# maturk/dn-splatter

Hardware: AMD Instinct MI355X
Metric: fwd+bwd frames/sec @1M Gaussians 1080p; HBM GB/s vs roofline (higher is better)
Workload: dtype f32; 1 GPU; c2: 1000000 random-init Gaussians, 1 camera/GPU 1920x1080, SH degree 3 + expected depth + per-Gaussian normals (7 channels, fused one-pass, post-ops in HIP), fx=fy=1200.0, orbit r=8, closed-form 3-NN scale init, random dense cotangents; scene=reference_init, N=1000000, pixels=2073600, bin_policy=deferred, parallelism=single GPU

## Files before the change

### dn-splatter_amd/csrc/binning.hip

```cpp

#include "splat_common.h"
#include "bin_ranges.h"

namespace {

constexpr int RS_THREADS = 256;
#ifndef DNS_RS_ITEMS_I
#define DNS_RS_ITEMS_I 16
#endif
constexpr int RS_ITEMS_I = DNS_RS_ITEMS_I;
#ifndef DNS_RS_ITEMS_N
#define DNS_RS_ITEMS_N 8
#endif
constexpr int RS_ITEMS_N = DNS_RS_ITEMS_N;
constexpr int RS_ITEMS_N_LARGE = 2 * DNS_RS_ITEMS_N;
constexpr int RS_LARGE_N = 1 << 22;
inline int rs_items_n(int N) { return N >= RS_LARGE_N ? RS_ITEMS_N_LARGE : RS_ITEMS_N; }
#ifndef DNS_TI_THREADS
#define DNS_TI_THREADS 512
#endif
constexpr int TI_THREADS = DNS_TI_THREADS;
constexpr int TI_ITEMS = RS_THREADS * RS_ITEMS_I / TI_THREADS;
static_assert(TI_THREADS * TI_ITEMS == RS_THREADS * RS_ITEMS_I && TI_THREADS % DNS_WAVE == 0 && TI_THREADS >= 256, "tile-pass chunk");
constexpr int RS_DIGITS = 256;

constexpr int SC_THREADS = 256;
constexpr int SC_ITEMS = 8;
constexpr int SC_CHUNK = SC_THREADS * SC_ITEMS;

__device__ __forceinline__ uint32_t lane_id() { return threadIdx.x & (DNS_WAVE - 1); }

__device__ __forceinline__ uint32_t wave_incl_scan(uint32_t v)
{
#pragma unroll
    for (int off = 1; off < DNS_WAVE; off <<= 1) {
        uint32_t t = __shfl_up(v, off, DNS_WAVE);
        if ((int)lane_id() >= off) v += t;
    }
    return v;
}

template <int NW = 4>
__device__ __forceinline__ uint32_t block_incl_scan(uint32_t v, uint32_t *lds_wave , uint32_t &total)
{
    const int w = threadIdx.x / DNS_WAVE;
    uint32_t inc = wave_incl_scan(v);
    if (lane_id() == DNS_WAVE - 1) lds_wave[w] = inc;
    __syncthreads();
    uint32_t base = 0, tot = 0;
#pragma unroll
    for (int i = 0; i < NW; ++i) {
        uint32_t s = lds_wave[i];
        if (i < w) base += s;
        tot += s;
    }
    total = tot;
    __syncthreads();
    return inc + base;
}
__device__ __forceinline__ uint32_t block_incl_scan_256(uint32_t v, uint32_t *lds_wave , uint32_t &total)
{
    return block_incl_scan<4>(v, lds_wave, total);
}

__device__ __forceinline__ uint32_t depth_key(const int32_t *__restrict__ radii, const float *__restrict__ depths, uint32_t g)
{
    return radii[g] > 0 ? __float_as_uint(depths[g]) : 0xFFFFFFFFu;
}

struct __align__(16) EmitRec {
    uint32_t gid;
    uint32_t start;
    uint32_t base_tile;
    uint32_t bw;
};
struct GenArgs {
    const EmitRec *__restrict__ jrec;
    const uint32_t *__restrict__ cum;
    const uint32_t *__restrict__ chunk_first;
    int N, tw;
    int exact;
    const uint32_t *__restrict__ n_ranked;
};

constexpr int gen_pad(int i) { return i + (i >> 5); }
// ... 325 lines not shown
        }
        const uint32_t prior = wave_cnt[w][d];
        const uint32_t below = __popcll(m & lt_mask);
        rnk[r] = prior + below;
        if (valid && below == 0) wave_cnt[w][d] = prior + __popcll(m);
    }
    __syncthreads();
    uint32_t n_out = n_valid;
    {
        const bool has_digit = threadIdx.x < ND;
        uint32_t cw[NW];
        uint32_t cnt = 0;
#pragma unroll
        for (int i = 0; i < NW; ++i) {
            cw[i] = has_digit ? wave_cnt[i][threadIdx.x] : 0u;
            cnt += cw[i];
        }
        uint32_t t2;
        const uint32_t linc = block_incl_scan<NW>(cnt, lds_wave, t2);
        const uint32_t ls = linc - cnt;
        if (FIRST) n_out = t2;
        if (has_digit) {
            dstart[threadIdx.x] = ls;
            uint32_t run = ls;
#pragma unroll
            for (int i = 0; i < NW; ++i) {
                wave_loc[i][threadIdx.x] = run;
                run += cw[i];
            }
        }
        const uint32_t tot = pre_tot;
        const uint32_t ginc = block_incl_scan<NW>(tot, lds_wave, t2);
        if (has_digit) gbase[threadIdx.x] = is_digit ? (ginc - tot) + pre_tab : 0u;
        if (FIRST && count_out && blockIdx.x == 0 && threadIdx.x == 0) *count_out = t2;
    }
    __syncthreads();
#pragma unroll
    for (int r = 0; r < ITEMS; ++r) {
        const uint32_t idx = wave_start + r * DNS_WAVE + lane;
        if (FIRST ? ((live >> r) & 1u) != 0u : idx < n) {
            const uint32_t d = (key[r] >> shift) & DMASK;
            const uint32_t lpos = wave_loc[w][d] + rnk[r];
            keys_s[lpos] = (K)key[r];
            vals_s[lpos] = val[r];
        }
    }
    __syncthreads();
    if constexpr (BOXG) {
        uint32_t dsts[ITEMS], vs[ITEMS];
        int2 bx[ITEMS];
#pragma unroll
        for (int r = 0; r < ITEMS; ++r) {
            const uint32_t i = min((uint32_t)(r * TH + threadIdx.x), n_out - 1u);
            const uint32_t d = ((uint32_t)keys_s[i] >> shift) & DMASK;
            dsts[r] = gbase[d] + (i - dstart[d]);
            vs[r] = vals_s[i];
        }
#pragma unroll
        for (int r = 0; r < ITEMS; ++r) bx[r] = box_in[vs[r]];
#pragma unroll
        for (int r = 0; r < ITEMS; ++r)
            if ((uint32_t)(r * TH + threadIdx.x) < n_out) {
                vals_out[dsts[r]] = vs[r];
                box_out[dsts[r]] = bx[r];
                tiles_out[dsts[r]] = ((uint32_t)bx[r].y & 0xffffu) * ((uint32_t)bx[r].y >> 16);
            }
        return;
    }
#pragma unroll
    for (int r = 0; r < ITEMS; ++r) {
        const uint32_t i = r * TH + threadIdx.x;
        if (i < n_out) {
            const uint32_t k = keys_s[i];
            const uint32_t d = (k >> shift) & DMASK;
            const uint32_t dst = gbase[d] + (i - dstart[d]);
            if (!LAST) keys_out[dst] = (K)k;
            vals_out[dst] = vals_s[i];
            if (LAST && (i == 0 || (uint32_t)keys_s[i - 1] != k)) atomicMin(&tile_first[k], (int32_t)dst);
            if (LAST && tile_end && (i + 1 == n_valid || (uint32_t)keys_s[i + 1] != k)) atomicMax(&tile_end[k], (int32_t)dst + 1);
        }
    }
}

template <bool BOXES>
__global__ __launch_bounds__(SC_THREADS) void scan_sums_kernel(int N, const uint32_t *__restrict__ n_ptr,
                                                               const uint32_t *__restrict__ order,
                                                               const int32_t *__restrict__ tiles,
                                                               uint32_t *__restrict__ sums, uint32_t *__restrict__ tiles_sorted,
                                                               const int2 *__restrict__ boxes = nullptr,
                                                               int2 *__restrict__ boxes_sorted = nullptr)
{
    __shared__ uint32_t lds_wave[4];
    const int n = (int)min(*n_ptr, (uint32_t)N);
    const int base = blockIdx.x * SC_CHUNK + threadIdx.x * SC_ITEMS;
    uint32_t s = 0;
    if (blockIdx.x * SC_CHUNK < n) {
        uint32_t o[SC_ITEMS], t[SC_ITEMS];
        [[maybe_unused]] int2 bx[SC_ITEMS];
#pragma unroll
        for (int i = 0; i < SC_ITEMS; ++i) o[i] = order[min(base + i, n - 1)];
#pragma unroll
        for (int i = 0; i < SC_ITEMS; ++i) {
            if (BOXES) {
                bx[i] = boxes[o[i]];
                t[i] = ((uint32_t)bx[i].y & 0xffffu) * ((uint32_t)bx[i].y >> 16);
            } else t[i] = (uint32_t)tiles[o[i]];
        }
#pragma unroll
        for (int i = 0; i < SC_ITEMS; ++i)
            if (base + i < n) {
                s += t[i];
                tiles_sorted[base + i] = t[i];
                if (BOXES) boxes_sorted[base + i] = bx[i];
            }
    }
    uint32_t tot;
    block_incl_scan_256(s, lds_wave, tot);
    if (threadIdx.x == 0) sums[blockIdx.x] = tot;
}

__global__ __launch_bounds__(SC_THREADS) void scan_sums_sorted_kernel(int N, const uint32_t *__restrict__ n_ptr,
                                                                      const uint32_t *__restrict__ tiles_sorted, uint32_t *__restrict__ sums)
{
    __shared__ uint32_t lds_wave[4];
    const int n = (int)min(*n_ptr, (uint32_t)N);
    const int base = blockIdx.x * SC_CHUNK + threadIdx.x * SC_ITEMS;
    uint32_t s = 0;
#pragma unroll
    for (int i = 0; i < SC_ITEMS; ++i)
        if (base + i < n) s += tiles_sorted[base + i];
    uint32_t tot;
    block_incl_scan_256(s, lds_wave, tot);
    if (threadIdx.x == 0) sums[blockIdx.x] = tot;
}

struct EmitPrep {
    EmitRec *__restrict__ jrec;
    uint32_t *__restrict__ chunk_first;
    int nb_chunks, chunk;
    int n_per_cam, tile_size, tw, th;
    const float *__restrict__ means2d;
    const int32_t *__restrict__ radii;
    const float4 *__restrict__ splats;
    const int2 *__restrict__ boxes;
    const int2 *__restrict__ boxes_sorted;
};

__device__ __forceinline__ void emit_record(const EmitPrep &ep, int N, uint32_t j, uint32_t gid, uint32_t start, uint32_t end)
{
    EmitRec r;
    r.gid = gid; r.start = start;
    const uint32_t cam_tiles = (ep.n_per_cam < N) ? (gid / (uint32_t)ep.n_per_cam) * (uint32_t)(ep.tw * ep.th) : 0u;
    if (ep.boxes) {
        const int2 b = ep.boxes_sorted ? ep.boxes_sorted[j] : ep.boxes[gid];
        r.bw = (uint32_t)b.y & 0xffffu;
        r.base_tile = (uint32_t)b.x + cam_tiles;
    } else {
        int x0, y0, x1, y1;
        if (ep.splats) {
            const float4 r0 = ep.splats[(size_t)gid * 4], r1 = ep.splats[(size_t)gid * 4 + 1];
            dns_snug_tile_bbox(r0.x, r0.y, r0.z, r0.w, r1.x, r1.y, (float)ep.radii[gid], ep.tile_size, ep.tw, ep.th, x0, y0, x1, y1);
        } else
            dns_tile_bbox(ep.means2d[2 * gid], ep.means2d[2 * gid + 1], (float)ep.radii[gid], ep.tile_size, ep.tw, ep.th, x0, y0, x1, y1);
        r.base_tile = (uint32_t)(y0 * ep.tw + x0) + cam_tiles;
        r.bw = (uint32_t)(x1 - x0);
    }
// ... 29 lines not shown
    for (int c = threadIdx.x; c < (int)blockIdx.x; c += SC_THREADS) before += sums[c];
    uint32_t tot_before;
    block_incl_scan_256(before, lds_wave, tot_before);
    uint32_t tot;
    uint32_t inc = block_incl_scan_256(s, lds_wave, tot);
    uint32_t run = tot_before + inc - s;
#pragma unroll
    for (int i = 0; i < SC_ITEMS; ++i) {
        int j = base + i;
        run += v[i];
        if (j < n) {
            cum[j] = run;
            if (j == n - 1) {
                *total_u32 = run; *total_i64 = (int64_t)run;
                if (total_max) atomicMax(reinterpret_cast<unsigned long long *>(total_max), (unsigned long long)run);
            }
        }
    }
}

__global__ __launch_bounds__(256) void emit_prep_kernel(int N, const uint32_t *__restrict__ n_ptr, const uint32_t *__restrict__ order,
                                                        const uint32_t *__restrict__ cum, EmitPrep ep)
{
    const uint32_t j = blockIdx.x * blockDim.x + threadIdx.x;
    if (j >= min(*n_ptr, (uint32_t)N)) return;
    const uint32_t end = cum[j], start = j ? cum[j - 1] : 0u;
    if (end > start) emit_record(ep, N, j, order[j], start, end);
}

constexpr int TO_THREADS = 1024;
__global__ __launch_bounds__(TO_THREADS) void tile_offsets_fill_kernel(int n_tiles, int32_t *__restrict__ offsets)
{
    __shared__ int32_t seg_min[TO_THREADS];
    const int total = n_tiles + 1;
    const int per = (total + TO_THREADS - 1) / TO_THREADS;
    const int lo = threadIdx.x * per, hi = min(lo + per, total);
    int32_t m = 0x7fffffff;
    for (int i = hi - 1; i >= lo; --i) m = min(m, offsets[i]);
    seg_min[threadIdx.x] = m;
    __syncthreads();
    for (int off = 1; off < TO_THREADS; off <<= 1) {
        const int32_t other = threadIdx.x + off < TO_THREADS ? seg_min[threadIdx.x + off] : 0x7fffffff;
        __syncthreads();
        seg_min[threadIdx.x] = min(seg_min[threadIdx.x], other);
        __syncthreads();
    }
    int32_t run = threadIdx.x + 1 < TO_THREADS ? seg_min[threadIdx.x + 1] : 0x7fffffff;
    for (int i = hi - 1; i >= lo; --i) {
        run = min(run, offsets[i]);
        offsets[i] = run;
    }
}

__global__ __launch_bounds__(256) void isect_ids_kernel(int n_tiles, int tile_bits, const int32_t *__restrict__ offsets,
                                                        const int32_t *__restrict__ flatten_ids,
                                                        const float *__restrict__ depths, int64_t *__restrict__ isect_ids,
                                                        int64_t cap)
{
    const int t = blockIdx.x;
    const int64_t cam = t / n_tiles, local = t % n_tiles;
    const int64_t hi = (cam << (32 + tile_bits)) | (local << 32);
    const int s = offsets[t], e = offsets[t + 1];
    for (int i = s + threadIdx.x; i < e && i < cap; i += blockDim.x) {
        const uint32_t bits = __float_as_uint(depths[flatten_ids[i]]);
        isect_ids[i] = hi | (int64_t)bits;
    }
}

constexpr int MAX_CHUNKS = (int)((0x80000000ull + RS_THREADS * RS_ITEMS_I - 1) / (RS_THREADS * RS_ITEMS_I));

struct BinWs {
    uint32_t *key_a, *key_b, *val_a, *val_b;
    uint32_t *cum;
    uint32_t *tiles_sorted;
    int2 *boxes_sorted;
    EmitRec *jrec;
    uint32_t *chunk_first;
    uint32_t *tab_n;
    uint32_t *totals;
    uint32_t *sums;
    uint32_t *total;
    uint32_t *status;
    uint32_t *n_ranked;
    uint32_t *tkey_b, *tval_b;
    uint32_t *tkey_c, *tval_c;
    uint32_t *tab_i;
    int nb_n, nb_i, nb_scan;
    size_t bytes;
};

inline size_t align_up(size_t v, size_t a) { return (v + a - 1) / a * a; }

BinWs carve(void *ws, int N, int64_t cap)
{
    BinWs b{};
    b.nb_n = (N + RS_THREADS * rs_items_n(N) - 1) / (RS_THREADS * rs_items_n(N));
    b.nb_i = (int)((cap + RS_THREADS * RS_ITEMS_I - 1) / (RS_THREADS * RS_ITEMS_I));
    b.nb_scan = (N + SC_CHUNK - 1) / SC_CHUNK;
    if (b.nb_n < 1) b.nb_n = 1;
    if (b.nb_i < 1) b.nb_i = 1;
    if (b.nb_scan < 1) b.nb_scan = 1;
    size_t off = 0;
    char *base = (char *)ws;
    auto take = [&](size_t elems) {
        uint32_t *p = (uint32_t *)(base + off);
        off += align_up(elems * sizeof(uint32_t), 256);
        return p;
    };
    size_t n = (size_t)(N > 0 ? N : 1), c = (size_t)(cap > 0 ? cap : 1);
    b.key_a = take(n); b.key_b = take(n); b.val_a = take(n); b.val_b = take(n);
    b.cum = take(n);
    b.tiles_sorted = take(n);
    b.boxes_sorted = reinterpret_cast<int2 *>(take(2 * n));
    b.jrec = reinterpret_cast<EmitRec *>(take(4 * n));
    b.chunk_first = take(MAX_CHUNKS);
    b.tab_n = take((size_t)RS_DIGITS * b.nb_n);
    b.totals = take((size_t)RS_DIGITS * SC_MAX_SEGS);
    b.sums = take(b.nb_scan);
    b.total = take(1);
    b.status = take(1);
    b.n_ranked = take(1);
    b.tkey_b = take(c); b.tval_b = take(c);
    b.tkey_c = take(c); b.tval_c = take(c);
    b.tab_i = take((size_t)RS_DIGITS * b.nb_i);
    b.bytes = off;
    return b;
}

int tile_bits(int n_tiles);

template <typename K, int ITEMS, int TH = RS_THREADS>
void radix_pass(hipStream_t stream, const K *ka, const uint32_t *va, K *kb, uint32_t *vb, const uint32_t *n_ptr,
                uint32_t n_cap, int shift, int dbits, uint32_t *table, uint32_t *totals, int nb, int32_t *tile_first = nullptr,
                const int32_t *radii = nullptr, const float *depths = nullptr, int32_t *init_offsets = nullptr, int n_tiles = 0,
                int32_t *tile_end = nullptr, const GenArgs *gen = nullptr, uint32_t *status = nullptr, uint32_t *count_out = nullptr,
                const int2 *box_in = nullptr, int2 *box_out = nullptr, uint32_t *tiles_out = nullptr)
{
    const uint32_t mask = (1u << dbits) - 1u;
    int segs, seg_len;
    scan_segments(nb, segs, seg_len);
    if (radii) {
        hipLaunchKernelGGL((radix_hist_kernel<K, ITEMS, true, false, TH>), dim3(nb), dim3(TH), 0, stream, ka, n_ptr, n_cap, shift, mask, table, nb, radii, depths);
        hipLaunchKernelGGL(radix_scan_kernel, dim3((1 << dbits) * segs), dim3(SC_THREADS), 0, stream, table, nb, totals, segs, seg_len);
        hipLaunchKernelGGL((radix_scatter_kernel<K, false, 8, ITEMS, true, false, TH>), dim3(nb), dim3(TH), 0, stream, ka, va, kb, vb,
                           n_ptr, n_cap, shift, table, totals, nb, tile_first, radii, depths, (int32_t *)nullptr, GenArgs{}, count_out,
                           (const int2 *)nullptr, (int2 *)nullptr, (uint32_t *)nullptr, segs, seg_len);
        return;
    }
    const GenArgs g = gen ? *gen : GenArgs{};
    if (gen && DNS_GEN_HIST_RANGES && shift == 0 && TH > RS_DIGITS)
        hipLaunchKernelGGL((radix_hist_ranges_kernel<ITEMS, (TH > RS_DIGITS ? TH : 2 * RS_DIGITS)>), dim3(nb), dim3(TH), 0, stream, n_ptr, n_cap, dbits,
                           table, nb, init_offsets, n_tiles, init_offsets ? tile_end : nullptr, g, status);
    else if (gen)
        hipLaunchKernelGGL((radix_hist_kernel<K, ITEMS, false, true, TH>), dim3(nb), dim3(TH), 0, stream, ka, n_ptr, n_cap, shift, mask,
                           table, nb, (const int32_t *)nullptr, (const float *)nullptr, init_offsets, n_tiles, init_offsets ? tile_end : nullptr, g, status);
    else
        hipLaunchKernelGGL((radix_hist_kernel<K, ITEMS, false, false, TH>), dim3(nb), dim3(TH), 0, stream, ka, n_ptr, n_cap, shift, mask, table, nb,
                           (const int32_t *)nullptr, (const float *)nullptr, init_offsets, n_tiles, init_offsets ? tile_end : nullptr, g, status);
    hipLaunchKernelGGL(radix_scan_kernel, dim3((1 << dbits) * segs), dim3(SC_THREADS), 0, stream, table, nb, totals, segs, seg_len);
    if constexpr (sizeof(K) == 4) {
        if (box_in && !gen && !tile_first && dbits == 8) {
            hipLaunchKernelGGL((radix_scatter_kernel<K, false, 8, ITEMS, false, false, TH, true>), dim3(nb), dim3(TH), 0, stream, ka, va, kb, vb,
                               n_ptr, n_cap, shift, table, totals, nb, tile_first, (const int32_t *)nullptr, (const float *)nullptr,
                               (int32_t *)nullptr, GenArgs{}, (uint32_t *)nullptr, box_in, box_out, tiles_out, segs, seg_len);
            return;
        }
    }
#define DNS_SCATTER3(B, L, G)                                                                                               \
    hipLaunchKernelGGL((radix_scatter_kernel<K, L, B, ITEMS, false, G, TH>), dim3(nb), dim3(TH), 0, stream, ka, va, kb, vb,    \
                       n_ptr, n_cap, shift, table, totals, nb, tile_first, (const int32_t *)nullptr, (const float *)nullptr, \
                       tile_end, g, (uint32_t *)nullptr, (const int2 *)nullptr, (int2 *)nullptr, (uint32_t *)nullptr, segs, seg_len)
#define DNS_SCATTER(B)                                                                                                      \
    do {                                                                                                                    \
        if (tile_first) { if (gen) DNS_SCATTER3(B, true, true); else DNS_SCATTER3(B, true, false); }                        \
        else { if (gen) DNS_SCATTER3(B, false, true); else DNS_SCATTER3(B, false, false); }                                 \
    } while (0)
    switch (dbits) {
        case 1: DNS_SCATTER(1); break;
        case 2: DNS_SCATTER(2); break;
        case 3: DNS_SCATTER(3); break;
        case 4: DNS_SCATTER(4); break;
        case 5: DNS_SCATTER(5); break;
        case 6: DNS_SCATTER(6); break;
        case 7: DNS_SCATTER(7); break;
        default: DNS_SCATTER(8); break;
    }
#undef DNS_SCATTER
#undef DNS_SCATTER3
}

template <typename K>
void emit_and_sort(hipStream_t stream, const dnsplat_bin_args *a, const BinWs &w, int tw, int th, int n_tiles, uint32_t cap)
{
    K *kb = reinterpret_cast<K *>(w.tkey_b), *kc = reinterpret_cast<K *>(w.tkey_c);
    uint32_t *vb = w.tval_b, *vc = w.tval_c;
    const int n_cam = a->n_cameras > 1 ? a->n_cameras : 1;
    const int bits = tile_bits(n_tiles);
    const int passes = (bits + 7) / 8;
    GenArgs g;
    g.jrec = w.jrec; g.cum = w.cum; g.chunk_first = w.chunk_first;
    g.N = a->N; g.tw = tw; g.n_ranked = w.n_ranked;
    g.exact = (tw <= 256 && (int64_t)n_cam * tw * th <= 65536) ? 1 : 0;
    const K *ka = nullptr;
    const uint32_t *va = nullptr;
// ... 47 lines not shown
    d.totals = take((size_t)RS_DIGITS * SC_MAX_SEGS);
    d.count = take(1);
    d.bytes = off;
    return d;
}

__global__ __launch_bounds__(256) void det_iota_kernel(const int64_t *__restrict__ n_isects, uint32_t cap, uint32_t *__restrict__ vals,
                                                       uint32_t *__restrict__ count)
{
    const uint32_t n = (uint32_t)min((int64_t)cap, max((int64_t)0, *n_isects));
    if (blockIdx.x == 0 && threadIdx.x == 0) *count = n;
    for (uint32_t i = blockIdx.x * blockDim.x + threadIdx.x; i < n; i += gridDim.x * blockDim.x) vals[i] = i;
}

__global__ __launch_bounds__(256) void det_reduce_kernel(const uint32_t *__restrict__ count, const uint32_t *__restrict__ keys,
                                                         const uint32_t *__restrict__ vals, const float *__restrict__ partials,
                                                         size_t cap, int n_records, float *__restrict__ v_splats)
{
    const uint32_t n = *count;
    const uint32_t i = (uint32_t)(((size_t)blockIdx.x * blockDim.x + threadIdx.x) >> 4);
    const int col = threadIdx.x & 15;
    if (i >= n) return;
    const uint32_t g = keys[i];
    if ((i > 0 && keys[i - 1] == g) || g >= (uint32_t)n_records) return;
    double acc = 0.0;
    for (uint32_t j = i; j < n && keys[j] == g; ++j) {
        const size_t e = vals[j];
        acc += (double)partials[e * DNS_REC + col];
        acc += (double)partials[(cap + e) * DNS_REC + col];
    }
    v_splats[(size_t)g * DNS_REC + col] = (float)acc;
}

}

extern "C" size_t dnsplat_det_workspace_bytes(int64_t capacity)
{
    if (capacity < 0) return 0;
    return det_carve(nullptr, capacity).bytes;
}

extern "C" int dnsplat_det_reduce(const dnsplat_det_args *a, dnsplat_stream_t stream_)
{
    if (!a || a->n_records < 0 || a->capacity < 0 || a->capacity > 0x7fffffffLL) return DNSPLAT_ERR_INVALID_ARG;
    if (a->capacity == 0 || a->n_records == 0) return DNSPLAT_OK;
    if (!a->n_isects || !a->flatten_ids || !a->partials || !a->v_splats || !a->workspace) return DNSPLAT_ERR_INVALID_ARG;
    if (a->workspace_bytes < det_carve(nullptr, a->capacity).bytes) return DNSPLAT_ERR_WORKSPACE;
    hipStream_t stream = (hipStream_t)stream_;
    const DetWs w = det_carve(a->workspace, a->capacity);
    const uint32_t cap = (uint32_t)a->capacity;
    hipLaunchKernelGGL(det_iota_kernel, dim3(1024), dim3(256), 0, stream, a->n_isects, cap, w.val_a, w.count);
    int bits = 1;
    while ((1ll << bits) < (long long)a->n_records) ++bits;
    const int passes = (bits + 7) / 8;
    const uint32_t *ka = reinterpret_cast<const uint32_t *>(a->flatten_ids);
    uint32_t *va = w.val_a, *kb = w.key_a, *vb = w.val_b;
    for (int pass = 0; pass < passes; ++pass) {
        radix_pass<uint32_t, RS_ITEMS_N>(stream, ka, va, kb, vb, w.count, cap, 8 * pass, 8, w.table, w.totals, w.nb);
        ka = kb; va = vb;
        kb = (kb == w.key_a) ? w.key_b : w.key_a;
        vb = (vb == w.val_b) ? w.val_a : w.val_b;
    }
    const size_t groups = (size_t)cap;
    hipLaunchKernelGGL(det_reduce_kernel, dim3((unsigned)((groups * 16 + 255) / 256)), dim3(256), 0, stream, w.count, ka, va, a->partials,
                       (size_t)a->capacity, a->n_records, a->v_splats);
    DNS_CHECK_LAUNCH();
    return DNSPLAT_OK;
}

extern "C" size_t dnsplat_bin_workspace_bytes(int32_t N, int64_t isect_capacity, int32_t n_tiles)
{
    (void)n_tiles;
    if (N < 0 || isect_capacity < 0) return 0;
    return carve(nullptr, N, isect_capacity).bytes;
}

extern "C" size_t dnsplat_bin_status_offset(int32_t N, int64_t isect_capacity)
{
    if (N < 0 || isect_capacity < 0) return 0;
    const BinWs w = carve(nullptr, N, isect_capacity);
    return (size_t)((char *)w.status - (char *)nullptr);
}

static int check_bin(const dnsplat_bin_args *a)
{
    if (!a) return DNSPLAT_ERR_INVALID_ARG;
    if (a->N < 0 || a->width <= 0 || a->height <= 0 || a->tile_size <= 0) return DNSPLAT_ERR_INVALID_ARG;
    if (a->n_cameras < 0 || (a->n_cameras > 1 && a->N % a->n_cameras != 0)) return DNSPLAT_ERR_INVALID_ARG;
    if (a->isect_capacity < 0 || a->isect_capacity > 0x7fffffffLL) return DNSPLAT_ERR_INVALID_ARG;
    if (!a->n_isects || !a->workspace) return DNSPLAT_ERR_INVALID_ARG;
    if (a->N > 0 && (!a->means2d || !a->radii || !a->depths || !a->tiles_per_gauss)) return DNSPLAT_ERR_INVALID_ARG;
    if (a->workspace_bytes < carve(nullptr, a->N, a->isect_capacity).bytes) return DNSPLAT_ERR_WORKSPACE;
    return DNSPLAT_OK;
}

extern "C" int dnsplat_bin_prepare(const dnsplat_bin_args *a, dnsplat_stream_t stream_)
{
    int rc = check_bin(a);
    if (rc != DNSPLAT_OK) return rc;
    hipStream_t stream = (hipStream_t)stream_;
    BinWs w = carve(a->workspace, a->N, a->isect_capacity);
    const int N = a->N;
    if (a->tight_tiles && !a->splats && !a->tile_boxes && N > 0) return DNSPLAT_ERR_INVALID_ARG;
    if (N == 0) {
        if (hipMemsetAsync(a->n_isects, 0, sizeof(int64_t), stream) != hipSuccess) return DNSPLAT_ERR_LAUNCH;
        if (hipMemsetAsync(w.total, 0, sizeof(uint32_t), stream) != hipSuccess) return DNSPLAT_ERR_LAUNCH;
    } else {
        const uint32_t n_u32 = (uint32_t)N;
        uint32_t *ka = w.key_a, *kb = w.key_b, *va = w.val_a, *vb = w.val_b;
        const int2 *boxes = reinterpret_cast<const int2 *>(a->tile_boxes);
        static const bool box_gather = [] { const char *e = getenv("DNSPLAT_BIN_BOX_GATHER"); return !(e && e[0] == '0'); }();
        const bool sorted_boxes = boxes && box_gather;
        static const bool box_fold = [] { const char *e = getenv("DNSPLAT_BIN_BOX_FOLD"); return !(e && e[0] == '0'); }();
        const bool fold = sorted_boxes && box_fold;
        for (int pass = 0; pass < 4; ++pass) {
            const int shift = 8 * pass;
            const bool fold_here = fold && pass == 3;
            if (rs_items_n(N) == RS_ITEMS_N_LARGE)
                radix_pass<uint32_t, RS_ITEMS_N_LARGE>(stream, ka, va, kb, vb, pass == 0 ? nullptr : w.n_ranked, n_u32, shift, 8, w.tab_n, w.totals,
                                                       w.nb_n, nullptr, pass == 0 ? a->radii : nullptr, pass == 0 ? a->depths : nullptr, nullptr, 0,
                                                       nullptr, nullptr, nullptr, pass == 0 ? w.n_ranked : nullptr,
                                                       fold_here ? boxes : nullptr, w.boxes_sorted, w.tiles_sorted);
            else
                radix_pass<uint32_t, RS_ITEMS_N>(stream, ka, va, kb, vb, pass == 0 ? nullptr : w.n_ranked, n_u32, shift, 8, w.tab_n, w.totals,
                                                 w.nb_n, nullptr, pass == 0 ? a->radii : nullptr, pass == 0 ? a->depths : nullptr, nullptr, 0,
                                                 nullptr, nullptr, nullptr, pass == 0 ? w.n_ranked : nullptr,
                                                 fold_here ? boxes : nullptr, w.boxes_sorted, w.tiles_sorted);
            uint32_t *t = ka; ka = kb; kb = t;
            t = va; va = vb; vb = t;
        }
        if (fold)
            hipLaunchKernelGGL(scan_sums_sorted_kernel, dim3(w.nb_scan), dim3(SC_THREADS), 0, stream, N, w.n_ranked, w.tiles_sorted, w.sums);
        else if (sorted_boxes)
            hipLaunchKernelGGL(scan_sums_kernel<true>, dim3(w.nb_scan), dim3(SC_THREADS), 0, stream, N, w.n_ranked, w.val_a, a->tiles_per_gauss,
                               w.sums, w.tiles_sorted, boxes, w.boxes_sorted);
        else
            hipLaunchKernelGGL(scan_sums_kernel<false>, dim3(w.nb_scan), dim3(SC_THREADS), 0, stream, N, w.n_ranked, w.val_a, a->tiles_per_gauss,
                               w.sums, w.tiles_sorted);
        EmitPrep ep;
        ep.jrec = w.jrec; ep.chunk_first = w.chunk_first; ep.nb_chunks = MAX_CHUNKS; ep.chunk = RS_THREADS * RS_ITEMS_I;
        ep.n_per_cam = N / (a->n_cameras > 1 ? a->n_cameras : 1);
        ep.tile_size = a->tile_size;
        ep.tw = dns_tiles_w(a->width, a->tile_size); ep.th = dns_tiles_h(a->height, a->tile_size);
        ep.means2d = a->means2d; ep.radii = a->radii;
        ep.splats = a->tight_tiles ? reinterpret_cast<const float4 *>(a->splats) : nullptr;
        ep.boxes = boxes;
        ep.boxes_sorted = sorted_boxes ? w.boxes_sorted : nullptr;
        hipLaunchKernelGGL(scan_final_kernel, dim3(w.nb_scan), dim3(SC_THREADS), 0, stream, N, w.n_ranked, w.val_a,
                           (const int32_t *)w.tiles_sorted, w.sums, w.cum, w.total, a->n_isects, a->n_isects_max);
        hipLaunchKernelGGL(emit_prep_kernel, dim3((N + 255) / 256), dim3(256), 0, stream, N, w.n_ranked, w.val_a, w.cum, ep);
        DNS_CHECK_LAUNCH();
    }
    if (a->n_isects_host) {
        if (hipMemcpyAsync(a->n_isects_host, a->n_isects, sizeof(int64_t), hipMemcpyDeviceToHost, stream) != hipSuccess)
            return DNSPLAT_ERR_LAUNCH;
    }
    return DNSPLAT_OK;
}

extern "C" int dnsplat_bin_emit_sort(const dnsplat_bin_args *a, dnsplat_stream_t stream_)
{
    int rc = check_bin(a);
    if (rc != DNSPLAT_OK) return rc;
    if (!a->tile_offsets || (a->isect_capacity > 0 && !a->flatten_ids)) return DNSPLAT_ERR_INVALID_ARG;
    if (a->tight_tiles && !a->splats && !a->tile_boxes && a->N > 0) return DNSPLAT_ERR_INVALID_ARG;
    hipStream_t stream = (hipStream_t)stream_;
    BinWs w = carve(a->workspace, a->N, a->isect_capacity);
    const int tw = dns_tiles_w(a->width, a->tile_size), th = dns_tiles_h(a->height, a->tile_size);
    const int64_t n_tiles64 = (int64_t)tw * th * (a->n_cameras > 1 ? a->n_cameras : 1);
    if (n_tiles64 > 0x7fffffffLL) return DNSPLAT_ERR_UNSUPPORTED;
    const int n_tiles = (int)n_tiles64;
    const uint32_t cap = (uint32_t)a->isect_capacity;
    if (a->N == 0 || cap == 0) {
        if (hipMemsetAsync(a->tile_offsets, 0, sizeof(int32_t) * (size_t)(n_tiles + 1), stream) != hipSuccess)
            return DNSPLAT_ERR_LAUNCH;
        if (a->tile_ends && hipMemsetAsync(a->tile_ends, 0, sizeof(int32_t) * (size_t)n_tiles, stream) != hipSuccess)
            return DNSPLAT_ERR_LAUNCH;
        return DNSPLAT_OK;
    }
    if (n_tiles <= 0x10000) emit_and_sort<uint16_t>(stream, a, w, tw, th, n_tiles, cap);
    else emit_and_sort<uint32_t>(stream, a, w, tw, th, n_tiles, cap);
    DNS_CHECK_LAUNCH();
    return DNSPLAT_OK;
}

extern "C" int dnsplat_bin_isect_ids(int32_t n_tiles, int32_t n_cameras, const int32_t *tile_offsets,
                                     const int32_t *flatten_ids, const float *depths, int64_t *isect_ids, int64_t capacity,
                                     dnsplat_stream_t stream)
{
    if (n_tiles <= 0 || n_cameras < 0 || !tile_offsets || !isect_ids) return DNSPLAT_ERR_INVALID_ARG;
    if (capacity == 0) return DNSPLAT_OK;
    if (!flatten_ids || !depths) return DNSPLAT_ERR_INVALID_ARG;
    const int n_cam = n_cameras > 1 ? n_cameras : 1;
    int tb = 0;
    while ((n_tiles >> tb) != 0) ++tb;
    hipLaunchKernelGGL(isect_ids_kernel, dim3(n_tiles * n_cam), dim3(256), 0, (hipStream_t)stream, n_tiles, tb, tile_offsets,
                       flatten_ids, depths, isect_ids, capacity);
    DNS_CHECK_LAUNCH();
    return DNSPLAT_OK;
}
```

Before: 476.1 frames/s.

## Sort depths via bucket partition and per-bucket LDS radix sort for mid-size N

For N below the large threshold, replaces the four global 8-bit radix passes over depth keys with a min/max bounds pass, a single histogram+scatter partition into depth buckets, and a per-bucket radix sort in shared memory that also gathers tile boxes. The aim is to cut global memory traffic and kernel launches of the full radix sort. Skewed depth distributions can overflow the LDS cap and fall back to slower in-global LSD passes inside one workgroup.

```diff
diff --git a/dn-splatter_amd/csrc/binning.hip b/dn-splatter_amd/csrc/binning.hip
--- a/dn-splatter_amd/csrc/binning.hip
+++ b/dn-splatter_amd/csrc/binning.hip
@@ -1,6 +1,9 @@
 
+#include <assert.h>
+#include <string.h>
 #include "splat_common.h"
 #include "bin_ranges.h"
+#include "depth_buckets.h"
 
 namespace {
 
@@ -492,6 +495,392 @@
     }
 }
 
+constexpr int DP_THREADS = 256;
+constexpr int DP_ITEMS = 16;
+constexpr int DP_CHUNK = DP_THREADS * DP_ITEMS;
+constexpr int DP_NW = DP_THREADS / DNS_WAVE;
+constexpr int DP_CAP = DNS_DP_CAP;
+constexpr int DP_BOUNDS_WGS = 1024;
+static_assert(DP_BOUNDS_WGS % DP_THREADS == 0, "the partials are reduced in rounds of one per thread");
+#ifndef DNS_DP_BBITS
+#define DNS_DP_BBITS 0
+#endif
+inline int dp_bbits(int N) { return DNS_DP_BBITS ? DNS_DP_BBITS : dns_depth_bucket_bits(N); }
+inline int dp_sub(int N) { const int s = (1 << dp_bbits(N)) >> 10; return s < 1 ? 1 : s; }
+inline int dp_bounds_wgs(int N)
+{
+    const int g = (N + DP_CHUNK - 1) / DP_CHUNK;
+    return g < 1 ? 1 : (g > DP_BOUNDS_WGS ? DP_BOUNDS_WGS : g);
+}
+
+__device__ __forceinline__ void dp_block_minmax(uint32_t &mn, uint32_t &mx, uint32_t *red )
+{
+#pragma unroll
+    for (int off = DNS_WAVE / 2; off > 0; off >>= 1) {
+        mn = min(mn, (uint32_t)__shfl_xor((int)mn, off, DNS_WAVE));
+        mx = max(mx, (uint32_t)__shfl_xor((int)mx, off, DNS_WAVE));
+    }
+    const int w = threadIdx.x / DNS_WAVE;
+    if (lane_id() == 0) { red[2 * w] = mn; red[2 * w + 1] = mx; }
+    __syncthreads();
+#pragma unroll
+    for (int i = 0; i < DP_NW; ++i) { mn = min(mn, red[2 * i]); mx = max(mx, red[2 * i + 1]); }
+    __syncthreads();
+}
+
+__global__ __launch_bounds__(DP_THREADS) void depth_bounds_kernel(const int32_t *__restrict__ radii, const float *__restrict__ depths,
+                                                                  uint32_t n, uint32_t *__restrict__ part)
+{
+    __shared__ uint32_t red[2 * DP_NW];
+    uint32_t mn = 0xFFFFFFFFu, mx = 0u;
+    constexpr int U = 4;
+    for (uint32_t i0 = blockIdx.x * (DP_THREADS * U) + threadIdx.x; i0 < n; i0 += gridDim.x * (DP_THREADS * U)) {
+        int32_t r[U];
+        uint32_t k[U];
+#pragma unroll
+        for (int u = 0; u < U; ++u) {
+            const uint32_t i = min(i0 + u * DP_THREADS, n - 1u);
+            r[u] = radii[i];
+            k[u] = __float_as_uint(depths[i]);
+        }
+#pragma unroll
+        for (int u = 0; u < U; ++u)
+            if (r[u] > 0) { mn = min(mn, k[u]); mx = max(mx, k[u]); }
+    }
+    dp_block_minmax(mn, mx, red);
+    if (threadIdx.x == 0) { part[2 * blockIdx.x] = mn; part[2 * blockIdx.x + 1] = mx; }
+}
+
+template <int BBITS>
+__global__ __launch_bounds__(DP_THREADS) void depth_part_hist_kernel(const int32_t *__restrict__ radii, const float *__restrict__ depths,
+                                                                     uint32_t n, const uint32_t *__restrict__ part, int n_part,
+                                                                     uint32_t *__restrict__ ks, uint32_t *__restrict__ table, int nb,
+                                                                     int sub)
+{
+    constexpr int NB = 1 << BBITS;
+    __shared__ uint32_t hist[NB];
+    __shared__ uint32_t red[2 * DP_NW];
+    uint32_t mn = 0xFFFFFFFFu, mx = 0u;
+    for (int i = threadIdx.x; i < n_part; i += DP_THREADS) { mn = min(mn, part[2 * i]); mx = max(mx, part[2 * i + 1]); }
+    for (int d = threadIdx.x; d < NB; d += DP_THREADS) hist[d] = 0u;
+    dp_block_minmax(mn, mx, red);
+    uint32_t kmin = 0u;
+    int shift = 0;
+    if (mn <= mx) { kmin = mn; shift = dns_depth_bucket_shift(mn, mx, BBITS); }
+    if (blockIdx.x == 0 && threadIdx.x == 0) { ks[0] = kmin; ks[1] = (uint32_t)shift; }
+    for (int c = 0; c < sub; ++c) {
+        const uint32_t base = (blockIdx.x * sub + c) * DP_CHUNK;
+        if (base >= n) break;
+        int32_t r[DP_ITEMS];
+        uint32_t k[DP_ITEMS];
+#pragma unroll
+        for (int i = 0; i < DP_ITEMS; ++i) {
+            const uint32_t idc = min(base + i * DP_THREADS + threadIdx.x, n - 1u);
+            r[i] = radii[idc];
+            k[i] = __float_as_uint(depths[idc]);
+        }
+#pragma unroll
+        for (int i = 0; i < DP_ITEMS; ++i)
+            if (base + i * DP_THREADS + threadIdx.x < n && r[i] > 0) atomicAdd(&hist[dns_depth_bucket(k[i], kmin, shift) & (NB - 1)], 1u);
+    }
+    __syncthreads();
+    for (int d = threadIdx.x; d < NB; d += DP_THREADS) table[(size_t)d * nb + blockIdx.x] = hist[d];
+}
+
+template <int BBITS>
+__global__ __launch_bounds__(DP_THREADS) void depth_part_scatter_kernel(
+    const int32_t *__restrict__ radii, const float *__restrict__ depths, uint32_t n, const uint32_t *__restrict__ ks,
+    uint2 *__restrict__ pairs_out, const uint32_t *__restrict__ table, const uint32_t *__restrict__ totals, int nb, int segs, int seg_len,
+    uint32_t *__restrict__ count_out, uint32_t *__restrict__ bucket_start, int sub)
+{
+    constexpr int NB = 1 << BBITS;
+    constexpr int DPT = NB / DP_THREADS;
+    static_assert(NB % DP_THREADS == 0 && DP_CHUNK <= 0xFFFF, "bucket scan layout / 16-bit chunk-local counts");
+    __shared__ __align__(4) uint16_t wave_cnt[DP_NW][NB];
+    __shared__ uint32_t gbase[NB];
+    __shared__ uint32_t lds_wave[DP_NW];
+    const uint32_t base0 = blockIdx.x * sub * DP_CHUNK;
+    if (base0 >= n) return;
+    const uint32_t kmin = ks[0];
+    const int shift = (int)ks[1];
+    const int w = threadIdx.x / DNS_WAVE;
+    const uint32_t lane = lane_id();
+    const uint64_t lt_mask = (lane == 0) ? 0ull : (~0ull >> (64 - lane));
+    {
+        uint32_t pre_tot[DPT], pre_tab[DPT];
+        const int my_seg = (int)blockIdx.x / seg_len;
+        uint32_t tsum = 0u;
+#pragma unroll
+        for (int q = 0; q < DPT; ++q) {
+            const int d = threadIdx.x * DPT + q;
+            pre_tab[q] = table[(size_t)d * nb + blockIdx.x];
+            pre_tot[q] = 0u;
+            for (int sg = 0; sg < segs; ++sg) {
+                const uint32_t v = totals[d * segs + sg];
+                pre_tot[q] += v;
+                if (sg < my_seg) pre_tab[q] += v;
+            }
+            tsum += pre_tot[q];
+        }
+        uint32_t total;
+        const uint32_t inc = block_incl_scan<DP_NW>(tsum, lds_wave, total);
+        uint32_t run = inc - tsum;
+#pragma unroll
+        for (int q = 0; q < DPT; ++q) {
+            const int d = threadIdx.x * DPT + q;
+            gbase[d] = run + pre_tab[q];
+            if (blockIdx.x == 0) bucket_start[d] = run;
+            run += pre_tot[q];
+        }
+        if (blockIdx.x == 0 && threadIdx.x == 0) { bucket_start[NB] = total; *count_out = total; }
+    }
+    for (int c = 0; c < sub; ++c) {
+        const uint32_t base = base0 + c * DP_CHUNK;
+        if (base >= n) break;
+        {
+            uint32_t *z = reinterpret_cast<uint32_t *>(&wave_cnt[0][0]);
+            for (int i = threadIdx.x; i < DP_NW * NB / 2; i += DP_THREADS) z[i] = 0u;
+        }
+        __syncthreads();
+        const uint32_t wave_start = base + w * (DNS_WAVE * DP_ITEMS);
+        uint32_t key[DP_ITEMS];
+        int32_t rad[DP_ITEMS];
+        uint16_t rnk[DP_ITEMS];
+#pragma unroll
+        for (int r = 0; r < DP_ITEMS; ++r) {
+            const uint32_t idc = min(wave_start + r * DNS_WAVE + lane, n - 1u);
+            rad[r] = radii[idc];
+            key[r] = __float_as_uint(depths[idc]);
+        }
+        uint32_t live = 0u;
+#pragma unroll
+        for (int r = 0; r < DP_ITEMS; ++r) {
+            const uint32_t idx = wave_start + r * DNS_WAVE + lane;
+            const bool valid = idx < n && rad[r] > 0;
+            live |= (valid ? 1u : 0u) << r;
+            const uint32_t d = valid ? (dns_depth_bucket(key[r], kmin, shift) & (NB - 1)) : 0u;
+            uint64_t m = dns_ballot(valid);
+#pragma unroll
+            for (int bit = 0; bit < BBITS; ++bit) {
+                const bool b = (d >> bit) & 1;
+                const uint64_t bal = dns_ballot(b);
+                m &= b ? bal : ~bal;
+            }
+            const uint32_t prior = wave_cnt[w][d];
+            const uint32_t below = __popcll(m & lt_mask);
+            rnk[r] = (uint16_t)(prior + below);
+            if (valid && below == 0) wave_cnt[w][d] = (uint16_t)(prior + __popcll(m));
+        }
+        __syncthreads();
+        uint32_t cnt[DPT];
+#pragma unroll
+        for (int q = 0; q < DPT; ++q) {
+            const int d = threadIdx.x * DPT + q;
+            uint32_t run = 0u;
+#pragma unroll
+            for (int i = 0; i < DP_NW; ++i) {
+                const uint32_t v = wave_cnt[i][d];
+                wave_cnt[i][d] = (uint16_t)run;
+                run += v;
+            }
+            cnt[q] = run;
+        }
+        __syncthreads();
+#pragma unroll
+        for (int r = 0; r < DP_ITEMS; ++r)
+            if ((live >> r) & 1u) {
+                const uint32_t d = dns_depth_bucket(key[r], kmin, shift) & (NB - 1);
+                const uint32_t dst = gbase[d] + wave_cnt[w][d] + rnk[r];
+                pairs_out[dst] = make_uint2(key[r], wave_start + r * DNS_WAVE + lane);
+            }
+        __syncthreads();
+#pragma unroll
+        for (int q = 0; q < DPT; ++q) gbase[threadIdx.x * DPT + q] += cnt[q];
+    }
+}
+
+__device__ __forceinline__ void dp_lsd_pass(const uint2 *src, uint2 *dst, uint32_t n, uint32_t kmin, int sh, int dbits,
+                                            uint32_t *dig_run , uint32_t (*wave_cnt)[256] , uint32_t *lds_wave)
+{
+    static_assert(DP_THREADS == 256, "one thread per digit");
+    const uint32_t mask = (1u << dbits) - 1u;
+    const int w = threadIdx.x / DNS_WAVE;
+    const uint32_t lane = lane_id();
+    const uint64_t lt_mask = (lane == 0) ? 0ull : (~0ull >> (64 - lane));
+    dig_run[threadIdx.x] = 0u;
+#pragma unroll
+    for (int i = 0; i < DP_NW; ++i) wave_cnt[i][threadIdx.x] = 0u;
+    __syncthreads();
+    for (uint32_t i = threadIdx.x; i < n; i += DP_THREADS) atomicAdd(&dig_run[((src[i].x - kmin) >> sh) & mask], 1u);
+    __syncthreads();
+    {
+        const uint32_t v = dig_run[threadIdx.x];
+        uint32_t tot;
+        const uint32_t inc = block_incl_scan<DP_NW>(v, lds_wave, tot);
+        dig_run[threadIdx.x] = inc - v;
+    }
+    __syncthreads();
+    for (uint32_t b0 = 0; b0 < n; b0 += DP_THREADS) {
+        const uint32_t i = b0 + threadIdx.x;
+        const bool valid = i < n;
+        const uint2 p = src[valid ? i : n - 1u];
+        const uint32_t d = valid ? (((p.x - kmin) >> sh) & mask) : 0u;
+        uint64_t m = dns_ballot(valid);
+#pragma unroll
+        for (int bit = 0; bit < 8; ++bit) {
+            const bool b = (d >> bit) & 1;
+            const uint64_t bal = dns_ballot(b);
+            m &= b ? bal : ~bal;
+        }
+        const uint32_t below = __popcll(m & lt_mask);
+        if (valid && below == 0) wave_cnt[w][d] = __popcll(m);
+        __syncthreads();
+        if (valid) {
+            uint32_t pos = dig_run[d] + below;
+#pragma unroll
+            for (int q = 0; q < DP_NW; ++q)
+                if (q < w) pos += wave_cnt[q][d];
+            dst[pos] = p;
+        }
+        __syncthreads();
+        {
+            uint32_t s = 0u;
+#pragma unroll
+            for (int q = 0; q < DP_NW; ++q) { s += wave_cnt[q][threadIdx.x]; wave_cnt[q][threadIdx.x] = 0u; }
+            dig_run[threadIdx.x] += s;
+        }
+        __syncthreads();
+    }
+}
+
+__device__ __forceinline__ void dp_store_bucket(const uint2 *res, uint32_t s, uint32_t n, uint32_t *__restrict__ vals_out,
+                                                const int2 *__restrict__ box_in, int2 *__restrict__ box_out,
+                                                uint32_t *__restrict__ tiles_out)
+{
+    constexpr int U = 4;
+    for (uint32_t i0 = threadIdx.x; i0 < n; i0 += U * DP_THREADS) {
+        uint32_t v[U];
+        int2 bx[U];
+#pragma unroll
+        for (int u = 0; u < U; ++u) v[u] = res[min(i0 + u * DP_THREADS, n - 1u)].y;
+        if (box_in) {
+#pragma unroll
+            for (int u = 0; u < U; ++u) bx[u] = box_in[v[u]];
+        }
+#pragma unroll
+        for (int u = 0; u < U; ++u) {
+            const uint32_t i = i0 + u * DP_THREADS;
+            if (i < n) {
+                vals_out[s + i] = v[u];
+                if (box_in) {
+                    box_out[s + i] = bx[u];
+                    tiles_out[s + i] = ((uint32_t)bx[u].y & 0xffffu) * ((uint32_t)bx[u].y >> 16);
+                }
+            }
+        }
+    }
+}
+
+__device__ __forceinline__ void dp_sort_in_lds(const uint2 *__restrict__ in, uint32_t n, uint32_t kmin, int passes, int dbits, uint2 *buf,
+                                               uint32_t *dig_start , uint32_t (*wave_cnt)[256] , uint32_t *lds_wave)
+{
+    constexpr int ITEMS = DP_CAP / DP_THREADS;
+    const int w = threadIdx.x / DNS_WAVE;
+    const uint32_t lane = lane_id();
+    const uint64_t lt_mask = (lane == 0) ? 0ull : (~0ull >> (64 - lane));
+    const int ipw = (int)((n + DP_THREADS - 1) / DP_THREADS);
+    const uint32_t first = (uint32_t)w * DNS_WAVE * ipw + lane;
+    const uint32_t mask = (1u << dbits) - 1u;
+    uint2 p[ITEMS];
+    uint32_t rnk[ITEMS];
+#pragma unroll
+    for (int r = 0; r < ITEMS; ++r)
+        if (r < ipw) p[r] = in[min(first + r * DNS_WAVE, n - 1u)];
+    if (passes == 0) {
+#pragma unroll
+        for (int r = 0; r < ITEMS; ++r)
+            if (r < ipw && first + r * DNS_WAVE < n) buf[first + r * DNS_WAVE] = p[r];
+    }
+    for (int pass = 0; pass < passes; ++pass) {
+        const int sh = pass * dbits;
+#pragma unroll
+        for (int i = 0; i < DP_NW; ++i) wave_cnt[i][threadIdx.x] = 0u;
+        __syncthreads();
+#pragma unroll
+        for (int r = 0; r < ITEMS; ++r)
+            if (r < ipw) {
+                const bool valid = first + r * DNS_WAVE < n;
+                const uint32_t d = valid ? (((p[r].x - kmin) >> sh) & mask) : 0u;
+                uint64_t m = dns_ballot(valid);
+#pragma unroll
+                for (int bit = 0; bit < 8; ++bit) {
+                    const bool b = (d >> bit) & 1;
+                    const uint64_t bal = dns_ballot(b);
+                    m &= b ? bal : ~bal;
+                }
+                const uint32_t prior = wave_cnt[w][d];
+                const uint32_t below = __popcll(m & lt_mask);
+                rnk[r] = prior + below;
+                if (valid && below == 0) wave_cnt[w][d] = prior + __popcll(m);
+            }
+        __syncthreads();
+        {
+            uint32_t cnt = 0u;
+#pragma unroll
+            for (int i = 0; i < DP_NW; ++i) {
+                const uint32_t c = wave_cnt[i][threadIdx.x];
+                wave_cnt[i][threadIdx.x] = cnt;
+                cnt += c;
+            }
+            uint32_t tot;
+            const uint32_t inc = block_incl_scan<DP_NW>(cnt, lds_wave, tot);
+            dig_start[threadIdx.x] = inc - cnt;
+        }
+        __syncthreads();
+#pragma unroll
+        for (int r = 0; r < ITEMS; ++r)
+            if (r < ipw && first + r * DNS_WAVE < n) {
+                const uint32_t d = ((p[r].x - kmin) >> sh) & mask;
+                buf[dig_start[d] + wave_cnt[w][d] + rnk[r]] = p[r];
+            }
+        __syncthreads();
+        if (pass + 1 < passes) {
+#pragma unroll
+            for (int r = 0; r < ITEMS; ++r)
+                if (r < ipw) p[r] = buf[min(first + r * DNS_WAVE, n - 1u)];
+        }
+    }
+    __syncthreads();
+}
+
+__global__ __launch_bounds__(DP_THREADS) void depth_bucket_sort_kernel(const uint32_t *__restrict__ ks,
+                                                                       const uint32_t *__restrict__ bucket_start, uint2 *pairs_a,
+                                                                       uint2 *pairs_b, uint32_t *__restrict__ vals_out,
+                                                                       const int2 *__restrict__ box_in, int2 *__restrict__ box_out,
+                                                                       uint32_t *__restrict__ tiles_out)
+{
+    __shared__ uint2 buf[DP_CAP];
+    __shared__ uint32_t dig_run[256];
+    __shared__ uint32_t wave_cnt[DP_NW][256];
+    __shared__ uint32_t lds_wave[DP_NW];
+    const uint32_t s = bucket_start[blockIdx.x], n = bucket_start[blockIdx.x + 1] - s;
+    if (n == 0) return;
+    const uint32_t kmin = ks[0];
+    const int shift = (int)ks[1];
+    const int passes = dns_depth_local_passes(shift), dbits = dns_depth_local_bits(shift);
+    if (n <= (uint32_t)DP_CAP) {
+        dp_sort_in_lds(pairs_a + s, n, kmin, passes, dbits, buf, dig_run, wave_cnt, lds_wave);
+        dp_store_bucket(buf, s, n, vals_out, box_in, box_out, tiles_out);
+    } else {
+        uint2 *src = pairs_a + s, *dst = pairs_b + s;
+        for (int p = 0; p < passes; ++p) {
+            dp_lsd_pass(src, dst, n, kmin, p * dbits, dbits, dig_run, wave_cnt, lds_wave);
+            uint2 *t = src; src = dst; dst = t;
+        }
+        dp_store_bucket(src, s, n, vals_out, box_in, box_out, tiles_out);
+    }
+}
+
 template <bool BOXES>
 __global__ __launch_bounds__(SC_THREADS) void scan_sums_kernel(int N, const uint32_t *__restrict__ n_ptr,
                                                                const uint32_t *__restrict__ order,
@@ -687,10 +1076,15 @@
     uint32_t *total;
     uint32_t *status;
     uint32_t *n_ranked;
+    uint32_t *dp_part;
+    uint32_t *dp_ks;
+    uint32_t *dp_start;
+    uint32_t *dp_tab;
+    uint32_t *dp_totals;
     uint32_t *tkey_b, *tval_b;
     uint32_t *tkey_c, *tval_c;
     uint32_t *tab_i;
-    int nb_n, nb_i, nb_scan;
+    int nb_n, nb_i, nb_scan, nb_p;
     size_t bytes;
 };
 
@@ -705,6 +1099,8 @@
     if (b.nb_n < 1) b.nb_n = 1;
     if (b.nb_i < 1) b.nb_i = 1;
     if (b.nb_scan < 1) b.nb_scan = 1;
+    b.nb_p = (N + DP_CHUNK * dp_sub(N) - 1) / (DP_CHUNK * dp_sub(N));
+    if (b.nb_p < 1) b.nb_p = 1;
     size_t off = 0;
     char *base = (char *)ws;
     auto take = [&](size_t elems) {
@@ -725,6 +1121,17 @@
     b.total = take(1);
     b.status = take(1);
     b.n_ranked = take(1);
+    {
+        const size_t B = (size_t)1 << dp_bbits(N), tab = B * b.nb_p;
+        uint32_t *q = b.chunk_first;
+        b.dp_part = q; q += 2 * DP_BOUNDS_WGS;
+        b.dp_ks = q; q += 64;
+        b.dp_start = q; q += align_up(B + 1, 64);
+        b.dp_totals = q; q += B * SC_MAX_SEGS;
+        const bool in_heads = (size_t)(q - b.chunk_first) + tab <= (size_t)MAX_CHUNKS;
+        b.dp_tab = in_heads ? q : b.key_a;
+        assert((size_t)(q - b.chunk_first) <= (size_t)MAX_CHUNKS && (in_heads || tab <= (size_t)(b.val_a - b.key_a)));
+    }
     b.tkey_b = take(c); b.tval_b = take(c);
     b.tkey_c = take(c); b.tval_c = take(c);
     b.tab_i = take((size_t)RS_DIGITS * b.nb_i);
@@ -938,6 +1345,17 @@
     return (size_t)((char *)w.status - (char *)nullptr);
 }
 
+static bool depth_sort_by_partition(int N)
+{
+    static const int pinned = [] {
+        const char *e = getenv("DNSPLAT_BIN_DEPTH_SORT");
+        return !e ? 0 : !strcmp(e, "radix4") ? 1 : !strcmp(e, "partition") ? 2 : 0;
+    }();
+    return pinned == 2 || (pinned == 0 && N < RS_LARGE_N);
+}
+
+extern "C" int dnsplat_bin_depth_route(int32_t N) { return depth_sort_by_partition(N) ? 1 : 0; }
+
 static int check_bin(const dnsplat_bin_args *a)
 {
     if (!a) return DNSPLAT_ERR_INVALID_ARG;
@@ -969,21 +1387,49 @@
         const bool sorted_boxes = boxes && box_gather;
         static const bool box_fold = [] { const char *e = getenv("DNSPLAT_BIN_BOX_FOLD"); return !(e && e[0] == '0'); }();
         const bool fold = sorted_boxes && box_fold;
-        for (int pass = 0; pass < 4; ++pass) {
-            const int shift = 8 * pass;
-            const bool fold_here = fold && pass == 3;
-            if (rs_items_n(N) == RS_ITEMS_N_LARGE)
-                radix_pass<uint32_t, RS_ITEMS_N_LARGE>(stream, ka, va, kb, vb, pass == 0 ? nullptr : w.n_ranked, n_u32, shift, 8, w.tab_n, w.totals,
-                                                       w.nb_n, nullptr, pass == 0 ? a->radii : nullptr, pass == 0 ? a->depths : nullptr, nullptr, 0,
-                                                       nullptr, nullptr, nullptr, pass == 0 ? w.n_ranked : nullptr,
-                                                       fold_here ? boxes : nullptr, w.boxes_sorted, w.tiles_sorted);
-            else
-                radix_pass<uint32_t, RS_ITEMS_N>(stream, ka, va, kb, vb, pass == 0 ? nullptr : w.n_ranked, n_u32, shift, 8, w.tab_n, w.totals,
-                                                 w.nb_n, nullptr, pass == 0 ? a->radii : nullptr, pass == 0 ? a->depths : nullptr, nullptr, 0,
-                                                 nullptr, nullptr, nullptr, pass == 0 ? w.n_ranked : nullptr,
-                                                 fold_here ? boxes : nullptr, w.boxes_sorted, w.tiles_sorted);
-            uint32_t *t = ka; ka = kb; kb = t;
-            t = va; va = vb; vb = t;
+        const bool radix4 = !depth_sort_by_partition(N);
+        if (!radix4) {
+            uint2 *pairs_a = reinterpret_cast<uint2 *>(w.jrec), *pairs_b = pairs_a + N;
+            const int n_part = dp_bounds_wgs(N), sub = dp_sub(N);
+            int segs, seg_len;
+            scan_segments(w.nb_p, segs, seg_len);
+            hipLaunchKernelGGL(depth_bounds_kernel, dim3(n_part), dim3(DP_THREADS), 0, stream, a->radii, a->depths, n_u32, w.dp_part);
+#define DNS_DEPTH_PARTITION(B)                                                                                                            \
+    do {                                                                                                                                  \
+        hipLaunchKernelGGL(depth_part_hist_kernel<B>, dim3(w.nb_p), dim3(DP_THREADS), 0, stream, a->radii, a->depths, n_u32, w.dp_part,   \
+                           n_part, w.dp_ks, w.dp_tab, w.nb_p, sub);                                                                       \
+        hipLaunchKernelGGL(radix_scan_kernel, dim3((1 << B) * segs), dim3(SC_THREADS), 0, stream, w.dp_tab, w.nb_p, w.dp_totals, segs,    \
+                           seg_len);                                                                                                      \
+        hipLaunchKernelGGL(depth_part_scatter_kernel<B>, dim3(w.nb_p), dim3(DP_THREADS), 0, stream, a->radii, a->depths, n_u32, w.dp_ks,  \
+                           pairs_a, w.dp_tab, w.dp_totals, w.nb_p, segs, seg_len, w.n_ranked, w.dp_start, sub);                           \
+    } while (0)
+            const int bbits = dp_bbits(N);
+            switch (bbits) {
+                case 9: DNS_DEPTH_PARTITION(9); break;
+                case 10: DNS_DEPTH_PARTITION(10); break;
+                case 11: DNS_DEPTH_PARTITION(11); break;
+                default: DNS_DEPTH_PARTITION(12); break;
+            }
+#undef DNS_DEPTH_PARTITION
+            hipLaunchKernelGGL(depth_bucket_sort_kernel, dim3(1 << bbits), dim3(DP_THREADS), 0, stream, w.dp_ks, w.dp_start, pairs_a, pairs_b,
+                               w.val_a, fold ? boxes : nullptr, w.boxes_sorted, w.tiles_sorted);
+        } else {
+            for (int pass = 0; pass < 4; ++pass) {
+                const int shift = 8 * pass;
+                const bool fold_here = fold && pass == 3;
+                if (rs_items_n(N) == RS_ITEMS_N_LARGE)
+                    radix_pass<uint32_t, RS_ITEMS_N_LARGE>(stream, ka, va, kb, vb, pass == 0 ? nullptr : w.n_ranked, n_u32, shift, 8, w.tab_n, w.totals,
+                                                           w.nb_n, nullptr, pass == 0 ? a->radii : nullptr, pass == 0 ? a->depths : nullptr, nullptr, 0,
+                                                           nullptr, nullptr, nullptr, pass == 0 ? w.n_ranked : nullptr,
+                                                           fold_here ? boxes : nullptr, w.boxes_sorted, w.tiles_sorted);
+                else
+                    radix_pass<uint32_t, RS_ITEMS_N>(stream, ka, va, kb, vb, pass == 0 ? nullptr : w.n_ranked, n_u32, shift, 8, w.tab_n, w.totals,
+                                                     w.nb_n, nullptr, pass == 0 ? a->radii : nullptr, pass == 0 ? a->depths : nullptr, nullptr, 0,
+                                                     nullptr, nullptr, nullptr, pass == 0 ? w.n_ranked : nullptr,
+                                                     fold_here ? boxes : nullptr, w.boxes_sorted, w.tiles_sorted);
+                uint32_t *t = ka; ka = kb; kb = t;
+                t = va; va = vb; vb = t;
+            }
         }
         if (fold)
             hipLaunchKernelGGL(scan_sums_sorted_kernel, dim3(w.nb_scan), dim3(SC_THREADS), 0, stream, N, w.n_ranked, w.tiles_sorted, w.sums);
diff --git a/dn-splatter_amd/csrc/depth_buckets.h b/dn-splatter_amd/csrc/depth_buckets.h
--- /dev/null
+++ b/dn-splatter_amd/csrc/depth_buckets.h
@@ -0,0 +1,41 @@
+#pragma once
+#include <stdint.h>
+
+#if defined(__HIPCC__)
+#define DNS_DB_HD __host__ __device__ __forceinline__
+#else
+#define DNS_DB_HD inline
+#endif
+
+#ifndef DNS_DP_CAP
+#define DNS_DP_CAP 4096
+#endif
+
+DNS_DB_HD int dns_depth_bucket_bits(int64_t N)
+{
+    int bits = 9;
+    while (bits < 12 && ((int64_t)1024 << bits) < N) ++bits;
+    return bits;
+}
+
+DNS_DB_HD int dns_bitlen_u32(uint32_t v)
+{
+    int n = 0;
+    while (v) { ++n; v >>= 1; }
+    return n;
+}
+
+DNS_DB_HD int dns_depth_bucket_shift(uint32_t kmin, uint32_t kmax, int bbits)
+{
+    const int s = dns_bitlen_u32(kmax - kmin) - bbits;
+    return s > 0 ? s : 0;
+}
+
+DNS_DB_HD uint32_t dns_depth_bucket(uint32_t k, uint32_t kmin, int shift) { return (k - kmin) >> shift; }
+
+DNS_DB_HD int dns_depth_local_passes(int shift) { return (shift + 7) / 8; }
+DNS_DB_HD int dns_depth_local_bits(int shift)
+{
+    const int p = dns_depth_local_passes(shift);
+    return p ? (shift + p - 1) / p : 0;
+}
```

Result: faster. 483.3 frames/s, median of 6 (+1.5%).
